# zj15001/PNP_ADMM_CNC_MRI

Measured on AMD Instinct MI355X. Metric: ADMM iterations/sec on 256x256 complex64 slices (batch=512), higher is better.
Workload: dtype f32

## Files before the change

### pnp_admm_cnc_mri_amd/csrc/kernels_slice256.hip

```cpp
#include "engine_host.h"
#include "fused_layout.h"
#include "slice_layout.h"
#include <math.h>
#include <stdio.h>
#include <stdlib.h>
#include <vector>

#ifndef SLICE_EARLY
#define SLICE_EARLY 1
#endif
#ifndef SLICE_PRIOSWAP
#define SLICE_PRIOSWAP 1
#endif
#ifndef SLICE_PRIOMASK
#define SLICE_PRIOMASK 6
#endif
#ifndef SLICE_YH_AUX
#define SLICE_YH_AUX 0
#endif
#ifndef SLICE_ST_AUX
#define SLICE_ST_AUX 0
#endif
#ifndef SLICE_PF
#define SLICE_PF 3
#endif

namespace pnp {

__device__ c32 g_tws[256];

struct SliceArgs {
    float* z;
    float* w;
    float* x;
    const c32* Yh;
    const uint32_t* Mh;
    const c32* Ys;
    const uint32_t* Ms;
    int first, B, iters;
    int slice_xor;
    int flip;
    int state_stride;
    int yh_stride;
    float scale, c;
    ProxParams prox;
    long long* prof;
};

constexpr int RP = 18;
constexpr int REGION = 16 * RP;
constexpr int WREG = 4 * REGION;
constexpr int SL_YS = SL_BUF + REGION;
constexpr int SL_LDS = SL_YS + 256 + 32;
static_assert(SL_WAVES * WREG <= SL_BUF, "wave regions must fit in the buffer they alias");
constexpr int SL4_XB = SL_WAVES * WREG;
constexpr int SL4_YS = SL4_XB + REGION;
constexpr int SL4_RES = SL4_YS + 256 + 32;
__device__ __forceinline__ int sl_lds_float(int set, int q) { return set == 0 ? sl_res_index(0, 0, q) : sl_res1_index(popc8(sl_units_lds(set) & ((1u << q) - 1)), 0, 0); }
constexpr int SL4_LDS = SL4_RES + SL_RES * 256 + SL_NLDS1 * 1024;
static_assert(SL_BUF4 <= SL4_XB && SL4_RES % 2 == 0 && SL4_LDS * 8 <= 160 * 1024, "four-pass LDS map");
template <int PROX> constexpr bool slice_four() { return PROX == 2; }
template <int PROX> constexpr bool slice_res() { return slice_four<PROX>() && SLICE_RESIDENT; }
__device__ __forceinline__ void lds_ld4(const float* p, float (&v)[4]) {
    const float4 q = *reinterpret_cast<const float4*>(p);
    v[0] = q.x; v[1] = q.y; v[2] = q.z; v[3] = q.w;
}
__device__ __forceinline__ void lds_st4(float* p, const float (&v)[4]) { *reinterpret_cast<float4*>(p) = make_float4(v[0], v[1], v[2], v[3]); }

__device__ __forceinline__ void wave_sync() {
    __builtin_amdgcn_fence(__ATOMIC_RELEASE, "wavefront");
    __builtin_amdgcn_wave_barrier();
    __builtin_amdgcn_fence(__ATOMIC_ACQUIRE, "wavefront");
#ifdef SLICE_SYNC_SCHED_BARRIER
    __builtin_amdgcn_sched_barrier(0);
#endif
}

__device__ __forceinline__ void prio_set(int wv, int set) {
#if SLICE_PRIOSWAP
    const bool older_high = (SLICE_PRIOMASK >> set) & 1;
    if (set == 0 || (((SLICE_PRIOMASK >> set) ^ (SLICE_PRIOMASK >> (set - 1))) & 1)) {
        asm volatile("" : "+s"(wv));
        if ((wv < 4) == older_high) __builtin_amdgcn_s_setprio(1); else __builtin_amdgcn_s_setprio(0);
    }
#endif
}

__device__ __forceinline__ int opaque(int v) {
    asm volatile("" : "+v"(v));
    return v;
}
typedef unsigned int u32x4 __attribute__((ext_vector_type(4)));
typedef unsigned int u32x2 __attribute__((ext_vector_type(2)));
typedef __amdgpu_buffer_rsrc_t bufrsrc;
__device__ __forceinline__ bufrsrc make_rsrc(const void* base, unsigned bytes) {
    return __builtin_amdgcn_make_buffer_rsrc(const_cast<void*>(base), 0, (int)bytes, 0x00020000);
}
__device__ __forceinline__ void ld4(bufrsrc r, int voff, int soff, float (&v)[4]) {
    const u32x4 q = __builtin_amdgcn_raw_buffer_load_b128(r, voff, soff, 16);
    v[0] = __uint_as_float(q.x); v[1] = __uint_as_float(q.y); v[2] = __uint_as_float(q.z); v[3] = __uint_as_float(q.w);
}
__device__ __forceinline__ void st4(bufrsrc r, int voff, int soff, const float (&v)[4]) {
    u32x4 q;
    q.x = __float_as_uint(v[0]); q.y = __float_as_uint(v[1]); q.z = __float_as_uint(v[2]); q.w = __float_as_uint(v[3]);
    __builtin_amdgcn_raw_buffer_store_b128(q, r, voff + soff, 0, SLICE_ST_AUX);
}
__device__ __forceinline__ c32 ldc(bufrsrc r, int voff, int soff) {
    const u32x2 q = __builtin_amdgcn_raw_buffer_load_b64(r, voff, soff, 0);
    return mk<float>(__uint_as_float(q.x), __uint_as_float(q.y));
}
struct SliceBufs {
    bufrsrc z, w, x;
    bufrsrc yh, mh, ys, ms;
};

__device__ __forceinline__ void pin(c32& v) { asm volatile("" : "+v"(v.x), "+v"(v.y)); }
__device__ __forceinline__ void mem_fence_compiler() { asm volatile("" ::: "memory"); }

__device__ __forceinline__ float dpp_lane_xor1(float v) {
    return __int_as_float(__builtin_amdgcn_mov_dpp(__float_as_int(v), 0xB1 , 0xF, 0xF, true));
}
__device__ __forceinline__ c32 dpp_lane_xor1(c32 v) { return mk<float>(dpp_lane_xor1(v.x), dpp_lane_xor1(v.y)); }

__device__ __forceinline__ float sub_partner(float a, float b) {
    float r;
    asm("v_subrev_f32_dpp %0, %1, %2 quad_perm:[1,0,3,2] row_mask:0xf bank_mask:0xf bound_ctrl:1" : "=v"(r) : "v"(b), "v"(a));
    return r;
}
__device__ __forceinline__ float add_partner(float a, float b) {
    float r;
    asm("v_add_f32_dpp %0, %1, %2 quad_perm:[1,0,3,2] row_mask:0xf bank_mask:0xf bound_ctrl:1" : "=v"(r) : "v"(b), "v"(a));
    return r;
}

__device__ __forceinline__ float abs_plus(float a, float w) {
    float r;
    asm("v_add_f32_e64 %0, |%1|, %2" : "=v"(r) : "v"(a), "v"(w));
    return r;
}

__device__ __forceinline__ f2 sub2(f2 a, f2 b) {
    f2 r;
    asm("v_pk_add_f32 %0, %1, %2 neg_lo:[0,1] neg_hi:[0,1]" : "=v"(r) : "v"(a), "v"(b));
    return r;
}


template <bool INV>
__device__ __forceinline__ void group_fft256(c32 (&ac)[16], const c32* twl, c32* region, int t) {
    typedef float f4 __attribute__((ext_vector_type(4)));
    const f4* tw4 = reinterpret_cast<const f4*>(twl + RP * t);
    f2* reg2 = reinterpret_cast<f2*>(region);
    f2 a[16];
#pragma unroll
    for (int k = 0; k < 16; ++k) a[k] = to2(ac[k]);
    dft16_pk<INV>(a);
    mem_fence_compiler();
#pragma unroll
    for (int m = 0; m < 4; ++m) {
        const f4 q = tw4[m];
        if (m) a[2 * m] = tmul_v<INV>(a[2 * m], k2(q.x, q.y));
        a[2 * m + 1] = tmul_v<INV>(a[2 * m + 1], k2(q.z, q.w));
    }
    mem_fence_compiler();
#pragma unroll
    for (int m = 4; m < 8; ++m) {
        const f4 q = tw4[m];
        a[2 * m] = tmul_v<INV>(a[2 * m], k2(q.x, q.y));
        a[2 * m + 1] = tmul_v<INV>(a[2 * m + 1], k2(q.z, q.w));
    }
#pragma unroll
    for (int k = 0; k < 16; ++k) reg2[k * RP + t] = a[k];
    wave_sync();
    const f4* row4 = reinterpret_cast<const f4*>(reg2 + t * RP);
#pragma unroll
    for (int m = 0; m < 8; ++m) {
        const f4 q = row4[m];
        a[2 * m] = k2(q.x, q.y);
        a[2 * m + 1] = k2(q.z, q.w);
    }
    wave_sync();
    dft16_pk<INV>(a);
#pragma unroll
    for (int k = 0; k < 16; ++k) ac[k] = from2(a[k]);
}

struct RowLoads {
    float z[8][4], w[8][4];
};
__device__ __forceinline__ int row_set_offset(int set, int wv) { return (32 * set + 4 * wv) * 2048; }
constexpr int ROW_QSTRIDE = 256;

template <int PROX, bool HAS_INV, int Q0, int Q1, bool RESW = false>
__device__ __forceinline__ void issue_row_loads(const SliceBufs& b, RowLoads& L, int soff, int voff, int qbase = 0, int set = 0, const float* resl = nullptr) {
#pragma unroll
    for (int q = qbase + Q0; q < qbase + Q1; ++q) {
        const int vo = voff + ROW_QSTRIDE * q, so = soff;
        const int home = RESW ? w_home(set, q) : W_HBM;
        if (home != W_HBM) {
            ld4(b.z, vo, so, L.z[q]);
            if (home == W_LDS) lds_ld4(resl + sl_lds_float(set, q), L.w[q]);
        } else if (PROX == 3) {
            ld4(b.w, vo, so, L.w[q]);
        } else if (PROX != 0 || !HAS_INV) {
            ld4(b.z, vo, so, L.z[q]);
            ld4(b.w, vo, so, L.w[q]);
        }
    }
}

__device__ __forceinline__ f2 clamp2(f2 a, float c) {
    return k2(__builtin_amdgcn_fmed3f(a.x, -c, c), __builtin_amdgcn_fmed3f(a.y, -c, c));
}
__device__ __forceinline__ f2 fma2(f2 a, f2 b, f2 c) { return __builtin_elementwise_fma(a, b, c); }
__device__ __forceinline__ f2 splat(float v) { return k2(v, v); }
template <int PROX>
__device__ __forceinline__ void prox_pair(f2 u, f2& z, f2& w, const ProxParams& pc) {
    if (PROX == 2) {
        const f2 cz = clamp2(z, pc.ib);
        const f2 t = fma2(splat(pc.c1), z, fma2(splat(pc.c2), u, splat(pc.c3) * cz));
        z = t - clamp2(t, pc.thr);
    } else {
        z = u - clamp2(u, pc.thr);
    }
    w = u - z;
}

template <bool HAS_INV, int PROX, bool HAS_FWD>
__device__ __forceinline__ void pointwise_q(const SliceBufs& b, const ProxParams& pc, int u_first, bool last,
                                            c32& a0, c32& a1, const float (&z_)[4], const float (&w_)[4], int vs,
                                            int home = W_HBM, float* resw = nullptr, float* wq = nullptr) {
    f2 z[2] = {k2(z_[0], z_[1]), k2(z_[2], z_[3])}, w[2] = {k2(w_[0], w_[1]), k2(w_[2], w_[3])};
#define SL_X_PLUS(a_, w_) (HAS_INV ? k2(abs_plus((a_).x, (w_).x), abs_plus((a_).y, (w_).y)) : (w_))
#define SL_ST4(buf, v) { const float q_[4] = {v[0].x, v[0].y, v[1].x, v[1].y}; st4(buf, vs, 0, q_); }
    if (PROX == 3) {
        f2 u[2];
#pragma unroll
        for (int jj = 0; jj < 2; ++jj) {
            if (!u_first) {
                asm volatile("");
                w[jj] = w[jj] - (w[jj] - clamp2(w[jj], pc.thr));
            }
            u[jj] = SL_X_PLUS(jj ? a1 : a0, w[jj]);
            z[jj] = u[jj] - clamp2(u[jj], pc.thr);
            w[jj] = u[jj] - z[jj];
        }
        if (!last) {
            SL_ST4(b.w, u);
        } else {
            SL_ST4(b.z, z);
            SL_ST4(b.w, w);
        }
    }
    if (PROX == 1 || PROX == 2) {
#pragma unroll
        for (int jj = 0; jj < 2; ++jj) prox_pair<PROX>(SL_X_PLUS(jj ? a1 : a0, w[jj]), z[jj], w[jj], pc);
        SL_ST4(b.z, z);
        if (home == W_LDS) { const float q_[4] = {w[0].x, w[0].y, w[1].x, w[1].y}; lds_st4(resw, q_); }
        else if (home == W_REG) { wq[0] = w[0].x; wq[1] = w[0].y; wq[2] = w[1].x; wq[3] = w[1].y; }
        else SL_ST4(b.w, w);
    }
#undef SL_ST4
#undef SL_X_PLUS
    if (HAS_FWD) {
        const f2 v0 = sub2(z[0], w[0]), v1 = sub2(z[1], w[1]);
        a0 = from2(v0);
        a1 = from2(v1);
    }
}

__device__ __forceinline__ void store_x_natural(const SliceBufs& b, const c32 (&a)[16], c32* wreg, int set, int wv, int lane) {
    const int g = lane >> 4, t = lane & 15;
    c32* region = wreg + g * REGION;
#pragma unroll
    for (int j = 0; j < 16; ++j) region[t + 16 * j] = mk<float>(fabsf(a[j].x), fabsf(a[j].y));
    wave_sync();
#pragma unroll
    for (int i = 0; i < 4; ++i) {
        const c32* cell = wreg + i * REGION + 4 * lane;
        const float4 c01 = *reinterpret_cast<const float4*>(cell);
        const float4 c23 = *reinterpret_cast<const float4*>(cell + 2);
        const int vs = 16 * lane + (2 * (32 * set + 4 * wv + i)) * 1024;
        const float xa[4] = {c01.x, c01.z, c23.x, c23.z}, xb[4] = {c01.y, c01.w, c23.y, c23.w};
        st4(b.x, vs, 0, xa);
        st4(b.x, vs + 1024, 0, xb);
    }
    wave_sync();
}

#ifndef SLICE_L1_PF
#define SLICE_L1_PF 8
#endif
template <int PROX> constexpr int row_pf() { return (PROX == 3) ? SLICE_L1_PF : SLICE_PF; }
__device__ __forceinline__ float* res_lane(float* res, int set, int wv, int lane) {
    return set == 0 ? res + sl_res_index(4 * wv + (lane >> 4), lane & 15, 0) : res + SL_RES * 512 + sl_res1_index(0, 4 * wv + (lane >> 4), lane & 15);
}
typedef float ResRegs[SL_NREG > 0 ? SL_NREG : 1][4];
template <int PROX, bool HAS_INV, bool RES = false>
__device__ __forceinline__ void row_phase_prefetch(const SliceBufs& b, RowLoads& L, int wv, int lane, float* res = nullptr) {
    issue_row_loads<PROX, HAS_INV, 0, row_pf<PROX>(), RES>(b, L, row_set_offset(0, wv), 2048 * (lane >> 4) + 16 * (lane & 15), 0, 0, RES ? res_lane(res, 0, wv, lane) : nullptr);
}
template <bool HAS_INV, int PROX, bool HAS_FWD, bool PRELOADED = false, bool RES = false>
__device__ __forceinline__ void row_phase(const SliceBufs& b, const ProxParams& pc, int u_first, bool last, c32 (&F)[SL_SETS][16],
                                          c32* wreg, const c32* twl, int wv, int lane, ResRegs& wr, RowLoads* pre = nullptr, float* res = nullptr) {
    const int g = lane >> 4, t = lane & 15;
    c32* region = wreg + g * REGION;
    const int voff = 2048 * g + 16 * t;
    float* const resl[2] = {RES ? res_lane(res, 0, wv, lane) : nullptr, RES && SL_NLDS1 ? res_lane(res, 1, wv, lane) : nullptr};
    constexpr bool RES_LOOP = RES && HAS_INV;
    constexpr int PF = row_pf<PROX>();
    RowLoads L;
    if (PRELOADED) L = *pre;
    else issue_row_loads<PROX, HAS_INV, 0, PF, RES_LOOP>(b, L, row_set_offset(0, wv), voff, 0, 0, resl[0]);
#pragma unroll
    for (int set = 0; set < SL_SETS; ++set) {
        c32 (&a)[16] = F[set];
        prio_set(wv, set);
        const int soff = row_set_offset(set, wv);
        if (HAS_INV) {
            group_fft256<true>(a, twl, region, t);
        }
        if (HAS_INV && last) store_x_natural(b, a, wreg, set, wv, lane);
        const int vs = voff + soff;
#pragma unroll
        for (int q = 0; q < 8; ++q) {
            const int home = RES ? w_home(set, q) : W_HBM;
            float* const rl = home == W_LDS ? resl[set] + sl_lds_float(set, q) : nullptr;
            float* const wq = wr[home == W_REG ? sl_reg_slot(set, q) : 0];
            if (q + PF < 8) issue_row_loads<PROX, HAS_INV, 0, 1, RES_LOOP>(b, L, soff, voff, q + PF, set, resl[set < 2 ? set : 0]);
            if (RES_LOOP && home != W_HBM) {
                pointwise_q<HAS_INV, PROX, HAS_FWD>(b, pc, u_first, last, a[2 * q], a[2 * q + 1], L.z[q], home == W_REG ? wr[sl_reg_slot(set, q)] : L.w[q],
                                                    vs + ROW_QSTRIDE * q, home, rl, wq);
            } else {
                if (home == W_LDS) lds_st4(rl, L.w[q]);
                if (home == W_REG) { wq[0] = L.w[q][0]; wq[1] = L.w[q][1]; wq[2] = L.w[q][2]; wq[3] = L.w[q][3]; }
                pointwise_q<HAS_INV, PROX, HAS_FWD>(b, pc, u_first, last, a[2 * q], a[2 * q + 1], L.z[q], L.w[q], vs + ROW_QSTRIDE * q);
            }
        }
        if (set + 1 < SL_SETS) issue_row_loads<PROX, HAS_INV, 0, PF, RES_LOOP>(b, L, row_set_offset(set + 1, wv), voff, 0, set + 1, resl[set + 1 < 2 ? set + 1 : 0]);
        if (HAS_FWD) {
            group_fft256<false>(a, twl, region, t);
        }
    }
}

__device__ __forceinline__ void resident_flush(const SliceBufs& b, float* res, const ResRegs& wr, int wv, int lane) {
#pragma unroll
    for (int set = 0; set < SL_SETS; ++set) {
        const int vs = 2048 * (lane >> 4) + 16 * (lane & 15) + row_set_offset(set, wv);
#pragma unroll
        for (int q = 0; q < 8; ++q) {
            const int home = w_home(set, q);
            if (home == W_LDS) {
                float v[4];
                lds_ld4(res_lane(res, set, wv, lane) + sl_lds_float(set, q), v);
                st4(b.w, vs + ROW_QSTRIDE * q, 0, v);
            } else if (home == W_REG) {
                st4(b.w, vs + ROW_QSTRIDE * q, 0, wr[sl_reg_slot(set, q)]);
            }
        }
    }
}

#define SL_PASS0_REGS(X, t)                                                                       \
    X(0, 0, (t)) X(1, 1, (t) + 16) X(2, 2, (t) + 32) X(3, 3, (t) + 48)                              \
    X(12, 8, ((t) ? SL_M + 64 - (t) : SL_M))                                                      \
    X(13, 13, SL_M + 48 - (t)) X(14, 14, SL_M + 32 - (t)) X(15, 15, SL_M + 16 - (t))
#define SL_PASS1_REGS(X, t)                                                                       \
    X(4, 4, (t)) X(5, 5, (t) + 16) X(6, 6, (t) + 32) X(7, 7, (t) + 48)                              \
    X(8, 12, ((t) ? SL_M + 64 - (t) : SL_M))                                                      \
    X(9, 9, SL_M + 48 - (t)) X(10, 10, SL_M + 32 - (t)) X(11, 11, SL_M + 16 - (t))

#define SL_PASS4_REGS(X, t, Q)                                                                    \
    X(2 * (Q), 2 * (Q), (t)) X(2 * (Q) + 1, 2 * (Q) + 1, (t) + 16)                                  \
    X(14 - 2 * (Q), ((Q) ? 16 - 2 * (Q) : 8), ((t) ? SL_M4 + 32 - (t) : SL_M4))                   \
    X(15 - 2 * (Q), 15 - 2 * (Q), SL_M4 + 16 - (t))

__device__ __forceinline__ void lds_put(c32* p, c32 v, bool swapped) {
    float* f = reinterpret_cast<float*>(p);
    if (swapped) { f[0] = v.y; f[1] = v.x; } else { *p = v; }
}
__device__ __forceinline__ c32 lds_get(const c32* p, bool swapped) {
    const float* f = reinterpret_cast<const float*>(p);
    return swapped ? mk<float>(f[1], f[0]) : *p;
}
template <int P, bool FOUR = false>
__device__ __forceinline__ void t_store_rows(const c32 (&F)[16], c32* rp, int t) {
#define SL_T1_STORE(ja, jb, slot) { lds_put(rp + (slot), t ? F[ja] : F[jb], (ja) >= 8); }
    if (FOUR) { SL_PASS4_REGS(SL_T1_STORE, t, P) } else if (P == 0) { SL_PASS0_REGS(SL_T1_STORE, t) } else { SL_PASS1_REGS(SL_T1_STORE, t) }
#undef SL_T1_STORE
}
template <int P, bool FOUR = false>
__device__ __forceinline__ void t_load_rows(c32 (&F)[16], const c32* rp, int t) {
#define SL_T2_LOAD(ja, jb, slot) { F[ja] = lds_get(rp + (slot), (ja) >= 8); }
    if (FOUR) { SL_PASS4_REGS(SL_T2_LOAD, t, P) } else if (P == 0) { SL_PASS0_REGS(SL_T2_LOAD, t) } else { SL_PASS1_REGS(SL_T2_LOAD, t) }
#undef SL_T2_LOAD
    if (FOUR && P == 3) {
        const c32 a8 = F[8];
        F[8] = t ? a8 : F[14];
        F[14] = t ? F[14] : F[12];
        F[12] = t ? F[12] : F[10];
        F[10] = t ? F[10] : a8;
    }
    if (!FOUR && P == 1) {
        const c32 a0 = F[8];
        F[8] = t ? a0 : F[12];
        F[12] = t ? F[12] : a0;
    }
}

template <bool MAYBE_PACKED, int PITCH = SL_P>
__device__ __forceinline__ void t1_read_col(c32 (&Gs)[16], const c32* buf, int off, int odd, bool packed) {
    int off_hi = off + 64 * PITCH;
    asm volatile("" : "+v"(off_hi));
    const c32 *col = buf + off, *col_hi = buf + off_hi;
#pragma unroll
    for (int jb = 0; jb < 16; jb += 8) {
        c32 own[8];
#pragma unroll
        for (int k = 0; k < 8; ++k) own[k] = jb ? col_hi[8 * k * PITCH] : col[8 * k * PITCH];
#pragma unroll
        for (int k = 0; k < 8; ++k) {
            c32 v = mk<float>(add_partner(own[k].x, own[k].y), sub_partner(own[k].y, own[k].x));
            if (MAYBE_PACKED) {
                const float oy = dpp_lane_xor1(own[k].y);
                const c32 raw = mk<float>(odd ? oy : own[k].x, odd ? own[k].x : oy);
                v = packed ? raw : v;
            }
            Gs[jb + k] = v;
            pin(Gs[jb + k]);
        }
    }
}
template <int P>
__device__ __forceinline__ void t1_pass(const c32 (&F)[SL_SETS][16], c32 (&G)[SL_SETS][16], c32* buf, int wv, int lane) {
    const int g = lane >> 4, t = lane & 15;
#pragma unroll
    for (int set = 0; set < SL_SETS; ++set) t_store_rows<P>(F[set], buf + (32 * set + 4 * wv + g) * SL_P, t);
    __syncthreads();
#pragma unroll
    for (int h = 0; h < 2; ++h) {
        const int cc = 32 * h + 4 * wv + g, odd = t & 1;
        const int off = (t >> 1) * SL_P + cc + (odd ? SL_M : 0);
        if (P == 0 && h == 0 && wv == 0) t1_read_col<true>(G[2 * P + h], buf, off, odd, cc == 0);
        else t1_read_col<false>(G[2 * P + h], buf, off, odd, false);
    }
    __syncthreads();
}

template <bool MAYBE_PACKED, int PITCH = SL_P>
__device__ __forceinline__ void t2_write_col(const c32 (&Gs)[16], c32* buf, int off, int odd, bool packed) {
    int off_hi = off + 64 * PITCH;
    asm volatile("" : "+v"(off_hi));
    c32 *col = buf + off, *col_hi = buf + off_hi;
#pragma unroll
    for (int j = 0; j < 16; ++j) {
        const c32 own = Gs[j];
        c32 v = mk<float>(sub_partner(own.x, own.y), add_partner(own.y, own.x));
        if (MAYBE_PACKED) {
            const c32 other = dpp_lane_xor1(own);
            const c32 raw = mk<float>(odd ? own.y : own.x, odd ? other.y : other.x);
            v = packed ? raw : v;
        }
        if (j < 8) col[8 * j * PITCH] = v; else col_hi[8 * (j - 8) * PITCH] = v;
    }
}
template <int P>
__device__ __forceinline__ void t2_pass(const c32 (&G)[SL_SETS][16], c32 (&F)[SL_SETS][16], c32* buf, int wv, int lane) {
    const int g = lane >> 4, t = lane & 15;
#pragma unroll
    for (int h = 0; h < 2; ++h) {
        const int cc = 32 * h + 4 * wv + g, odd = t & 1;
        const int off = (t >> 1) * SL_P + cc + (odd ? SL_M : 0);
        if (P == 0 && h == 0 && wv == 0) t2_write_col<true>(G[2 * P + h], buf, off, odd, cc == 0);
        else t2_write_col<false>(G[2 * P + h], buf, off, odd, false);
    }
    __syncthreads();
#pragma unroll
    for (int set = 0; set < SL_SETS; ++set) t_load_rows<P>(F[set], buf + (32 * set + 4 * wv + g) * SL_P, t);
    __syncthreads();
}

template <int Q>
__device__ __forceinline__ void t1_pass4(const c32 (&F)[SL_SETS][16], c32 (&G)[SL_SETS][16], c32* buf, int wv, int lane) {
    const int g = lane >> 4, t = lane & 15;
#pragma unroll
    for (int set = 0; set < SL_SETS; ++set) t_store_rows<Q, true>(F[set], buf + (32 * set + 4 * wv + g) * SL_P4, t);
    __syncthreads();
    const int cc = 4 * wv + g, odd = t & 1;
    const int off = (t >> 1) * SL_P4 + cc + (odd ? SL_M4 : 0);
    if (Q == 0 && wv == 0) t1_read_col<true, SL_P4>(G[Q], buf, off, odd, cc == 0);
    else t1_read_col<false, SL_P4>(G[Q], buf, off, odd, false);
    __syncthreads();
}
template <int Q>
__device__ __forceinline__ void t2_pass4(const c32 (&G)[SL_SETS][16], c32 (&F)[SL_SETS][16], c32* buf, int wv, int lane) {
    const int g = lane >> 4, t = lane & 15;
    const int cc = 4 * wv + g, odd = t & 1;
    const int off = (t >> 1) * SL_P4 + cc + (odd ? SL_M4 : 0);
    if (Q == 0 && wv == 0) t2_write_col<true, SL_P4>(G[Q], buf, off, odd, cc == 0);
    else t2_write_col<false, SL_P4>(G[Q], buf, off, odd, false);
    __syncthreads();
#pragma unroll
    for (int set = 0; set < SL_SETS; ++set) t_load_rows<Q, true>(F[set], buf + (32 * set + 4 * wv + g) * SL_P4, t);
    __syncthreads();
}

struct ColLoads {
    c32 yh[16];
    uint32_t code;
};
__device__ __forceinline__ void issue_col_loads(const SliceBufs& b, ColLoads& Y, int set, int wv, int lane) {
    const int ybase = (set * 8 + wv) * 8192;
    Y.code = __builtin_amdgcn_raw_buffer_load_b32(b.mh, 4 * lane, (set * 8 + wv) * 64 * 4, 0);
#pragma unroll
    for (int jp = 0; jp < 8; ++jp) {
        const u32x4 q = __builtin_amdgcn_raw_buffer_load_b128(b.yh, 16 * lane + 1024 * (jp & 3), ybase + 4096 * (jp >> 2), SLICE_YH_AUX);
        Y.yh[2 * jp] = mk<float>(__uint_as_float(q.x), __uint_as_float(q.y));
        Y.yh[2 * jp + 1] = mk<float>(__uint_as_float(q.z), __uint_as_float(q.w));
    }
}

__device__ __forceinline__ float code_byte(unsigned m, int byte) {
    float r;
    if (byte == 0) asm("v_cvt_f32_ubyte0 %0, %1" : "=v"(r) : "v"(m));
    else if (byte == 1) asm("v_cvt_f32_ubyte1 %0, %1" : "=v"(r) : "v"(m));
    else if (byte == 2) asm("v_cvt_f32_ubyte2 %0, %1" : "=v"(r) : "v"(m));
    else asm("v_cvt_f32_ubyte3 %0, %1" : "=v"(r) : "v"(m));
    return r;
}
__device__ __forceinline__ void blend_set(c32 (&a)[16], const c32 (&yh)[16], unsigned code, float cs, float chs, float os) {
    const unsigned m[4] = {code & 0x03030303u, (code >> 2) & 0x03030303u, (code >> 4) & 0x03030303u, (code >> 6) & 0x03030303u};
#pragma unroll
    for (int j = 0; j < 16; j += 2) {
        const f2 cf = k2(code_byte(m[j & 3], j >> 2), code_byte(m[(j & 3) + 1], j >> 2));
        const f2 A2 = fma2(splat(-chs), cf, splat(os));
        a[j] = from2(fma2(A2.xx, to2(a[j]), splat(cs) * to2(yh[j])));
        a[j + 1] = from2(fma2(A2.yy, to2(a[j + 1]), splat(cs) * to2(yh[j + 1])));
    }
}

__device__ __forceinline__ void col_phase(const SliceBufs& b, float cdc, float scale, c32 (&G)[SL_SETS][16], c32* wreg, c32* ysl, const c32* twl, int wv, int lane) {
    const int g = lane >> 4, t = lane & 15;
    c32* region = wreg + g * REGION;
    const float cs = cdc * scale, chs = 0.5f * cdc * scale;
    ColLoads Y;
    issue_col_loads(b, Y, 0, wv, lane);
    if (wv == 0) {
        __builtin_amdgcn_raw_ptr_buffer_load_lds(b.ys, ysl, 16, 16 * lane, 0, 0, 0);
        __builtin_amdgcn_raw_ptr_buffer_load_lds(b.ys, ysl + 128, 16, 16 * lane, 1024, 0, 0);
        __builtin_amdgcn_raw_ptr_buffer_load_lds(b.ms, ysl + 256, 4, 4 * lane, 0, 0, 0);
    }
#pragma unroll
    for (int set = 0; set < SL_SETS; ++set) {
        c32 (&a)[16] = G[set];
        prio_set(wv, set);
        group_fft256<false>(a, twl, region, t);
        if (set == 0 && wv == 0 && g == 0) {
#pragma unroll
            for (int j = 0; j < 16; ++j) region[t + 16 * j] = a[j];
            region[256 + t] = a[0];
            wave_sync();
            const uint32_t code_b = reinterpret_cast<const uint32_t*>(ysl + 256)[t];
            const c32* mirror = region + (16 - t);
            const unsigned ma[4] = {Y.code & 0x03030303u, (Y.code >> 2) & 0x03030303u, (Y.code >> 4) & 0x03030303u, (Y.code >> 6) & 0x03030303u};
            const unsigned mb[4] = {code_b & 0x03030303u, (code_b >> 2) & 0x03030303u, (code_b >> 4) & 0x03030303u, (code_b >> 6) & 0x03030303u};
#pragma unroll
            for (int j = 0; j < 16; ++j) {
                const c32 gm = mirror[16 * (15 - j)];
                const c32 A = blend_scaled_f(unpack_a(a[j], gm), Y.yh[j], code_byte(ma[j & 3], j >> 2), cs, chs, scale);
                const c32 Bv = blend_scaled_f(unpack_b(a[j], gm), ysl[t + 16 * j], code_byte(mb[j & 3], j >> 2), cs, chs, scale);
                a[j] = repack_p(A, Bv);
            }
            wave_sync();
        } else {
            blend_set(a, Y.yh, Y.code, cs, 0.5f * chs, 0.5f * scale);
        }
        if (set + 1 < SL_SETS) issue_col_loads(b, Y, set + 1, wv, lane);
        group_fft256<true>(a, twl, region, t);
    }
}

template <int PROX>
__global__ __launch_bounds__(512) void k_slice(SliceArgs p) {
    constexpr bool FOUR = slice_four<PROX>(), RES = slice_res<PROX>();
    __shared__ __attribute__((aligned(16))) c32 lds[FOUR ? SL4_LDS : SL_LDS];
    const int tid = threadIdx.x, lane = tid & 63;
    const int wv = __builtin_amdgcn_readfirstlane(tid >> 6);
    c32* twl = lds + (FOUR ? SL4_XB : SL_BUF);
    c32* ysl = lds + (FOUR ? SL4_YS : SL_YS);
    float* res = RES ? reinterpret_cast<float*>(lds + SL4_RES) : nullptr;
    if (tid < 256) twl[RP * (tid >> 4) + (tid & 15)] = g_tws[((tid >> 4) * (tid & 15)) & 255];
    c32* wreg = lds + wv * WREG;
    __syncthreads();
    for (int sb = blockIdx.x; sb < p.B; sb += gridDim.x) {
        const int sx = ((sb ^ p.slice_xor) < p.B) ? (sb ^ p.slice_xor) : sb;
        const int slice = p.first + (p.flip ? p.B - 1 - sx : sx);
        const size_t so = (size_t)slice * p.state_stride;
        SliceBufs b;
        b.z = make_rsrc(p.z + so, 65536 * 4); b.w = make_rsrc(p.w + so, 65536 * 4); b.x = make_rsrc(p.x + (size_t)slice * 65536, 65536 * 4);
        b.yh = make_rsrc(p.Yh + (size_t)slice * p.yh_stride, YH3_SLICE * 8); b.mh = make_rsrc(p.Mh + (size_t)slice * MH3_SLICE, MH3_SLICE * 4);
        b.ys = make_rsrc(p.Ys + (size_t)slice * 256, 256 * 8); b.ms = make_rsrc(p.Ms + (size_t)slice * 16, 16 * 4);
        c32 F[SL_SETS][16];
        ResRegs wres;
#ifdef SLICE_PROF
        long long* prof = (p.prof && tid == 0 && sb == (int)blockIdx.x) ? p.prof + (size_t)slice * (2 + 6 * p.iters) : nullptr;
#define SL_STAMP() if (prof) *prof++ = wall_clock64()
#else
#define SL_STAMP()
#endif
        SL_STAMP();
        row_phase<false, 0, true, false, RES>(b, p.prox, 1, false, F, wreg, twl, wv, opaque(lane), wres, nullptr, res);
        SL_STAMP();
        for (int it = 0; it < p.iters; ++it) {
            c32 G[SL_SETS][16];
            __syncthreads();
            SL_STAMP();
            if (FOUR) {
                t1_pass4<0>(F, G, lds, wv, opaque(lane));
                t1_pass4<1>(F, G, lds, wv, opaque(lane));
                t1_pass4<2>(F, G, lds, wv, opaque(lane));
                t1_pass4<3>(F, G, lds, wv, opaque(lane));
            } else {
                t1_pass<0>(F, G, lds, wv, opaque(lane));
                t1_pass<1>(F, G, lds, wv, opaque(lane));
            }
#ifdef SLICE_PROF_CLOCK
            if (prof) *prof++ = (long long)__builtin_readcyclecounter();
#else
            SL_STAMP();
#endif
            col_phase(b, p.c, p.scale, G, wreg, ysl, twl, wv, opaque(lane));
            SL_STAMP();
            __syncthreads();
            SL_STAMP();
            if (FOUR) {
                t2_pass4<0>(G, F, lds, wv, opaque(lane));
                t2_pass4<1>(G, F, lds, wv, opaque(lane));
                t2_pass4<2>(G, F, lds, wv, opaque(lane));
            } else {
                t2_pass<0>(G, F, lds, wv, opaque(lane));
            }
#if SLICE_EARLY
            RowLoads L0;
            row_phase_prefetch<PROX, true, RES>(b, L0, wv, opaque(lane), res);
#endif
            if (FOUR) t2_pass4<3>(G, F, lds, wv, opaque(lane));
            else t2_pass<1>(G, F, lds, wv, opaque(lane));
            SL_STAMP();
            const int u_first = (it == 0);
#if SLICE_EARLY
            row_phase<true, PROX, true, true, RES>(b, p.prox, u_first, it + 1 == p.iters, F, wreg, twl, wv, opaque(lane), wres, &L0, res);
#else
            row_phase<true, PROX, true, false, RES>(b, p.prox, u_first, it + 1 == p.iters, F, wreg, twl, wv, opaque(lane), wres, nullptr, res);
#endif
            SL_STAMP();
        }
        if (RES) resident_flush(b, res, wres, wv, opaque(lane));
        __syncthreads();
    }
}

constexpr int SP_P = 17;
__global__ __launch_bounds__(256) void k_sprepare(const c32* y, const uint8_t* mask_bank, const int32_t* mask_id,
                                                  c32* Yh, uint32_t* Mh, c32* Ys, uint32_t* Ms, int yh_stride) {
    __shared__ c32 yd[256 * SP_P], ym[256 * SP_P];
    __shared__ uint8_t md[256 * SP_P], mm[256 * SP_P];
    const int tid = threadIdx.x, m = blockIdx.x, slice = blockIdx.y;
    const int mid = mask_id ? mask_id[slice] : 0;
    const c32* ys = y + (size_t)slice * 65536;
    const uint8_t* ms = mask_bank + (size_t)mid * 65536;
    const int ncol = (m == 8) ? 1 : 16;
#pragma unroll 4
    for (int i = 0; i < 16; ++i) {
        const int idx = tid + 256 * i, r = idx >> 4, c = idx & 15;
        if (c < ncol) {
            const int k2 = 16 * m + c, k2m = (256 - k2) & 255;
            yd[r * SP_P + c] = ys[r * 256 + k2];
            md[r * SP_P + c] = ms[r * 256 + k2];
            ym[r * SP_P + c] = ys[r * 256 + k2m];
            mm[r * SP_P + c] = ms[r * 256 + k2m];
        }
    }
    __syncthreads();
    auto entry = [&](int k1, int c, c32& yh) -> int {
        const int r2 = (256 - k1) & 255;
        const int m1 = md[k1 * SP_P + c] != 0, m2 = mm[r2 * SP_P + c] != 0;
        const c32 y1 = yd[k1 * SP_P + c], y2 = ym[r2 * SP_P + c];
        yh = mk<float>(0.5f * ((m1 ? y1.x : 0.f) + (m2 ? y2.x : 0.f)), 0.5f * ((m1 ? y1.y : 0.f) - (m2 ? y2.y : 0.f)));
        return m1 + m2;
    };
    if (m == 8) {
        c32 yh;
        const int code = entry(tid, 0, yh);
        Ys[(size_t)slice * 256 + tid] = yh;
        __shared__ int codes[256];
        codes[tid] = code;
        __syncthreads();
        if (tid < 16) {
            uint32_t v = 0;
#pragma unroll
            for (int jj = 0; jj < 16; ++jj) v |= (uint32_t)codes[tid + 16 * jj] << (2 * jj);
            Ms[slice * 16 + tid] = v;
        }
        return;
    }
    const int set = m >> 1;
#pragma unroll 4
    for (int i = 0; i < 16; ++i) {
        const int o = tid + 256 * i, blk = o >> 10, e = o & 1023;
        const int jp = e >> 7, lane = (e >> 1) & 63, j = 2 * jp + (e & 1);
        const int g = lane >> 4, t = lane & 15, wv = 4 * (m & 1) + blk;
        c32 yh;
        (void)entry(t + 16 * j, 4 * blk + g, yh);
        Yh[(size_t)slice * yh_stride + yh3_index(0, set, j, wv, lane)] = yh;
    }
    {
        const int blk = tid >> 6, lane = tid & 63, g = lane >> 4, t = lane & 15, wv = 4 * (m & 1) + blk;
        uint32_t v = 0;
#pragma unroll
        for (int j = 0; j < 16; ++j) {
            c32 yh;
            v |= (uint32_t)entry(t + 16 * j, 4 * blk + g, yh) << (2 * j);
        }
        Mh[mh3_index(slice, set, wv, lane)] = v;
    }
}

template <bool TO_SLICE>
__global__ __launch_bounds__(128) void k_state_order(const float* sz, const float* sw, float* dz, float* dw, int src_stride, int dst_stride) {
    __shared__ float tile[2][2048];
    const size_t sbase = (size_t)blockIdx.y * src_stride + (size_t)blockIdx.x * 2048, dbase = (size_t)blockIdx.y * dst_stride + (size_t)blockIdx.x * 2048;
    const float4* pz = reinterpret_cast<const float4*>(sz + sbase);
    const float4* pw = reinterpret_cast<const float4*>(sw + sbase);
    float4* qz = reinterpret_cast<float4*>(dz + dbase);
    float4* qw = reinterpret_cast<float4*>(dw + dbase);
    float4 vz[4], vw[4];
#pragma unroll
    for (int u = 0; u < 4; ++u) { vz[u] = pz[threadIdx.x + 128 * u]; vw[u] = pw[threadIdx.x + 128 * u]; }
#pragma unroll
    for (int u = 0; u < 4; ++u) {
        const int i = threadIdx.x + 128 * u, row = i >> 6, n0 = 4 * (i & 63);
        const float az[4] = {vz[u].x, vz[u].y, vz[u].z, vz[u].w}, aw[4] = {vw[u].x, vw[u].y, vw[u].z, vw[u].w};
#pragma unroll
        for (int k = 0; k < 4; ++k) {
            const int at = TO_SLICE ? (int)sl_state_index(row, n0 + k) : 4 * i + k;
            tile[0][at] = az[k];
            tile[1][at] = aw[k];
        }
    }
    __syncthreads();
#pragma unroll
    for (int u = 0; u < 4; ++u) {
        const int i = threadIdx.x + 128 * u, row = i >> 6, n0 = 4 * (i & 63);
        float oz[4], ow[4];
#pragma unroll
        for (int k = 0; k < 4; ++k) {
            const int at = TO_SLICE ? 4 * i + k : (int)sl_state_index(row, n0 + k);
            oz[k] = tile[0][at];
            ow[k] = tile[1][at];
        }
        qz[i] = make_float4(oz[0], oz[1], oz[2], oz[3]);
        qw[i] = make_float4(ow[0], ow[1], ow[2], ow[3]);
    }
}

struct Slice256 {
    int Bmax = 0, cus = 0;
    int flip = 0;
    int pad = 0, yh_pad = 0;
    float* zs = nullptr;
    float* ws = nullptr;
    float* zprev = nullptr;
    c32* Yh = nullptr;
    uint32_t* Mh = nullptr;
    c32* Ys = nullptr;
    uint32_t* Ms = nullptr;
    SideQueues queues;
};

int slice256_cus(const Slice256* f) { return f && f->cus > 0 ? f->cus : 256; }

hipError_t slice256_state_order(Slice256* f, hipStream_t s, float* z, float* w, int B, bool to_slice) {
    if (B <= 0) return hipSuccess;
    if (f && f->pad > 0) {
        if (to_slice) hipLaunchKernelGGL(k_state_order<true>, dim3(32, B), dim3(128), 0, s, z, w, f->zs, f->ws, 65536, 65536 + f->pad);
        else          hipLaunchKernelGGL(k_state_order<false>, dim3(32, B), dim3(128), 0, s, f->zs, f->ws, z, w, 65536 + f->pad, 65536);
    } else {
        if (to_slice) hipLaunchKernelGGL(k_state_order<true>, dim3(32, B), dim3(128), 0, s, z, w, z, w, 65536, 65536);
        else          hipLaunchKernelGGL(k_state_order<false>, dim3(32, B), dim3(128), 0, s, z, w, z, w, 65536, 65536);
    }
    return hipGetLastError();
}

hipError_t slice256_trace_snapshot(Slice256* f, hipStream_t s, const float* z, int B) {
    const size_t stride = 65536 + (size_t)f->pad;
    if (B > f->Bmax) return hipErrorInvalidValue;
    if (!f->zprev) { hipError_t e = hipMalloc((void**)&f->zprev, (size_t)f->Bmax * stride * sizeof(float)); if (e != hipSuccess) return e; }
    return hipMemcpyAsync(f->zprev, f->pad > 0 ? f->zs : z, (size_t)B * stride * sizeof(float), hipMemcpyDeviceToDevice, s);
}
hipError_t slice256_residuals(Slice256* f, hipStream_t s, const float* x, const float* z, const float* w, const uint8_t* gt, int B,
                              double* partial, unsigned* counter, double* out) {
    if (!f->zprev || B > f->Bmax) return hipErrorInvalidValue;
    return launch_residuals<float>(s, x, f->pad > 0 ? f->zs : z, f->zprev, f->pad > 0 ? f->ws : w, gt, 0, B, 65536, 65536 + (size_t)f->pad, true,
                                   partial, counter, out);
}

// ... 115 lines not shown
```

### pnp_admm_cnc_mri_amd/csrc/slice_layout.h

```cpp
#pragma once
#include <stddef.h>
#include <stdint.h>
#include "fft16.h"

namespace pnp {

constexpr int SL_P = 132;
constexpr int SL_M = 66;
constexpr int SL_BUF = 128 * SL_P;

PNP_HD int sl_pass(int k) { return (k < 64 || k > 192 || k == 128) ? 0 : 1; }
PNP_HD int sl_slot(int k) {
    if (k < 64) return k;
    if (k == 128) return SL_M;
    if (k > 192) return SL_M + 256 - k;
    if (k < 128) return k - 64;
    return SL_M + 192 - k;
}
constexpr int SL_P4 = 68;
constexpr int SL_M4 = 34;
constexpr int SL_BUF4 = 128 * SL_P4;
PNP_HD int sl_pass4(int k) { return k == 128 ? 0 : k < 128 ? (k >> 5) : ((256 - k) >> 5); }
PNP_HD int sl_slot4(int k) { return k == 128 ? SL_M4 : k < 128 ? (k & 31) : SL_M4 + ((256 - k) & 31); }
constexpr int SL_WAVES = 8, SL_SETS = 4;
constexpr int SL_RES = 32;
PNP_HD int sl_res_index(int r, int t, int q) { return 512 * r + 64 * q + 4 * t; }
constexpr int SL_RES1 = 2;
PNP_HD int sl_res1_index(int u, int rr, int t) { return 2048 * u + 64 * rr + 4 * t; }
#ifndef SLICE_RESIDENT
#define SLICE_RESIDENT 1
#endif
#ifndef SLICE_UNITS_LDS1
#define SLICE_UNITS_LDS1 0x03
#endif
#ifndef SLICE_UNITS_REG
#define SLICE_UNITS_REG 0x03000000
#endif
constexpr int popc8(unsigned m) { int n = 0; for (int i = 0; i < 8; ++i) n += (m >> i) & 1; return n; }
constexpr unsigned sl_units_lds(int set) { return SLICE_RESIDENT == 0 ? 0u : set == 0 ? 0xFFu : (SLICE_RESIDENT == 1 && set == 1) ? (SLICE_UNITS_LDS1 & 0xFFu) : 0u; }
constexpr unsigned sl_units_reg(int set) { return SLICE_RESIDENT == 1 && set < SL_SETS ? ((unsigned)SLICE_UNITS_REG >> (8 * set)) & 0xFFu & ~sl_units_lds(set) : 0u; }
enum { W_HBM = 0, W_LDS = 1, W_REG = 2 };
constexpr int w_home(int set, int q) { return ((sl_units_lds(set) >> q) & 1) ? W_LDS : ((sl_units_reg(set) >> q) & 1) ? W_REG : W_HBM; }
constexpr int sl_reg_slot(int set, int q) {
    int n = 0;
    for (int s = 0; s < set; ++s) n += popc8(sl_units_reg(s));
    return n + (set < SL_SETS ? popc8(sl_units_reg(set) & ((1u << q) - 1)) : 0);
}
constexpr int SL_NREG = sl_reg_slot(SL_SETS, 0);
constexpr int SL_NLDS1 = popc8(sl_units_lds(1));
static_assert(SL_NLDS1 <= SL_RES1, "the second resident region holds SL_RES1 units");

PNP_HD int sl_unit(int set, int wv, int lane) { return 32 * set + 4 * wv + (lane >> 4); }

constexpr size_t YH3_SLICE = 4 * 16 * 8 * 64;
constexpr size_t MH3_SLICE = 4 * 8 * 64;
PNP_HD size_t yh3_index(int slice, int set, int j, int wv, int lane) {
    return (size_t)slice * YH3_SLICE + ((((size_t)set * 8 + wv) * 8 + (j >> 1)) * 64 + lane) * 2 + (j & 1);
}
PNP_HD size_t mh3_index(int slice, int set, int wv, int lane) { return (size_t)slice * MH3_SLICE + (((size_t)set * 8 + wv) * 64 + lane); }

PNP_HD size_t sl_state_index(int row, int n) {
    return (size_t)(row >> 1) * 512 + 64 * (n >> 5) + 4 * (n & 15) + 2 * ((n >> 4) & 1) + (row & 1);
}


}
```

Measured before the change: 11210.

## Shrink LDS exchange buffers to free space for more resident state units

The four-pass kernel now does its per-wave FFT transposes and the x store through float-split (real then imaginary) exchange regions, and runs the inter-phase transposes in two half-passes over a 64-row buffer. This roughly halves the LDS footprint of the scratch buffers. The freed LDS holds more of the per-slice w state as resident units (7 instead of 2 in the second region), so less state travels to and from HBM each iteration. The cost is extra wave syncs and block barriers per transpose, plus scalar rather than vector LDS accesses.

```diff
diff --git a/pnp_admm_cnc_mri_amd/csrc/kernels_slice256.hip b/pnp_admm_cnc_mri_amd/csrc/kernels_slice256.hip
--- a/pnp_admm_cnc_mri_amd/csrc/kernels_slice256.hip
+++ b/pnp_admm_cnc_mri_amd/csrc/kernels_slice256.hip
@@ -53,12 +53,8 @@
 constexpr int SL_YS = SL_BUF + REGION;
 constexpr int SL_LDS = SL_YS + 256 + 32;
 static_assert(SL_WAVES * WREG <= SL_BUF, "wave regions must fit in the buffer they alias");
-constexpr int SL4_XB = SL_WAVES * WREG;
-constexpr int SL4_YS = SL4_XB + REGION;
-constexpr int SL4_RES = SL4_YS + 256 + 32;
 __device__ __forceinline__ int sl_lds_float(int set, int q) { return set == 0 ? sl_res_index(0, 0, q) : sl_res1_index(popc8(sl_units_lds(set) & ((1u << q) - 1)), 0, 0); }
-constexpr int SL4_LDS = SL4_RES + SL_RES * 256 + SL_NLDS1 * 1024;
-static_assert(SL_BUF4 <= SL4_XB && SL4_RES % 2 == 0 && SL4_LDS * 8 <= 160 * 1024, "four-pass LDS map");
+static_assert(REGION * 8 == SL2_TW_BYTES && (256 + 32) * 8 == SL2_YS_BYTES && SL2_END % 8 == 0, "tables of the LDS map");
 template <int PROX> constexpr bool slice_four() { return PROX == 2; }
 template <int PROX> constexpr bool slice_res() { return slice_four<PROX>() && SLICE_RESIDENT; }
 __device__ __forceinline__ void lds_ld4(const float* p, float (&v)[4]) {
@@ -146,7 +142,8 @@
 }
 
 
-template <bool INV>
+typedef __attribute__((address_space(3))) float lds_float;
+template <bool INV, bool SPLIT = false>
 __device__ __forceinline__ void group_fft256(c32 (&ac)[16], const c32* twl, c32* region, int t) {
     typedef float f4 __attribute__((ext_vector_type(4)));
     const f4* tw4 = reinterpret_cast<const f4*>(twl + RP * t);
@@ -169,17 +166,31 @@
         a[2 * m] = tmul_v<INV>(a[2 * m], k2(q.x, q.y));
         a[2 * m + 1] = tmul_v<INV>(a[2 * m + 1], k2(q.z, q.w));
     }
-#pragma unroll
-    for (int k = 0; k < 16; ++k) reg2[k * RP + t] = a[k];
-    wave_sync();
-    const f4* row4 = reinterpret_cast<const f4*>(reg2 + t * RP);
-#pragma unroll
-    for (int m = 0; m < 8; ++m) {
-        const f4 q = row4[m];
-        a[2 * m] = k2(q.x, q.y);
-        a[2 * m + 1] = k2(q.z, q.w);
-    }
-    wave_sync();
+    if (SPLIT) {
+        float* rf = reinterpret_cast<float*>(region);
+        const volatile lds_float* row = (const volatile lds_float*)(rf + sl_xw(t, 0));
+#pragma unroll
+        for (int h = 0; h < 2; ++h) {
+#pragma unroll
+            for (int k = 0; k < 16; ++k) rf[sl_xw(k, t)] = h ? a[k].y : a[k].x;
+            wave_sync();
+#pragma unroll
+            for (int k = 0; k < 16; ++k) { if (h) a[k].y = row[k]; else a[k].x = row[k]; }
+            wave_sync();
+        }
+    } else {
+#pragma unroll
+        for (int k = 0; k < 16; ++k) reg2[k * RP + t] = a[k];
+        wave_sync();
+        const f4* row4 = reinterpret_cast<const f4*>(reg2 + t * RP);
+#pragma unroll
+        for (int m = 0; m < 8; ++m) {
+            const f4 q = row4[m];
+            a[2 * m] = k2(q.x, q.y);
+            a[2 * m + 1] = k2(q.z, q.w);
+        }
+        wave_sync();
+    }
     dft16_pk<INV>(a);
 #pragma unroll
     for (int k = 0; k < 16; ++k) ac[k] = from2(a[k]);
@@ -269,8 +280,27 @@
     }
 }
 
+template <bool SPLIT = false>
 __device__ __forceinline__ void store_x_natural(const SliceBufs& b, const c32 (&a)[16], c32* wreg, int set, int wv, int lane) {
     const int g = lane >> 4, t = lane & 15;
+    if (SPLIT) {
+        float* wf = reinterpret_cast<float*>(wreg);
+        float* rf = wf + g * SL_XREGION;
+#pragma unroll
+        for (int h = 0; h < 2; ++h) {
+#pragma unroll
+            for (int j = 0; j < 16; ++j) rf[t + 16 * j] = fabsf(h ? a[j].y : a[j].x);
+            wave_sync();
+#pragma unroll
+            for (int i = 0; i < 4; ++i) {
+                float v[4];
+                lds_ld4(wf + i * SL_XREGION + 4 * lane, v);
+                st4(b.x, 16 * lane + (2 * (32 * set + 4 * wv + i) + h) * 1024, 0, v);
+            }
+            wave_sync();
+        }
+        return;
+    }
     c32* region = wreg + g * REGION;
 #pragma unroll
     for (int j = 0; j < 16; ++j) region[t + 16 * j] = mk<float>(fabsf(a[j].x), fabsf(a[j].y));
@@ -300,11 +330,11 @@
 __device__ __forceinline__ void row_phase_prefetch(const SliceBufs& b, RowLoads& L, int wv, int lane, float* res = nullptr) {
     issue_row_loads<PROX, HAS_INV, 0, row_pf<PROX>(), RES>(b, L, row_set_offset(0, wv), 2048 * (lane >> 4) + 16 * (lane & 15), 0, 0, RES ? res_lane(res, 0, wv, lane) : nullptr);
 }
-template <bool HAS_INV, int PROX, bool HAS_FWD, bool PRELOADED = false, bool RES = false>
+template <bool HAS_INV, int PROX, bool HAS_FWD, bool PRELOADED = false, bool RES = false, bool SPLIT = false>
 __device__ __forceinline__ void row_phase(const SliceBufs& b, const ProxParams& pc, int u_first, bool last, c32 (&F)[SL_SETS][16],
                                           c32* wreg, const c32* twl, int wv, int lane, ResRegs& wr, RowLoads* pre = nullptr, float* res = nullptr) {
     const int g = lane >> 4, t = lane & 15;
-    c32* region = wreg + g * REGION;
+    c32* region = SPLIT ? reinterpret_cast<c32*>(reinterpret_cast<float*>(wreg) + g * SL_XREGION) : wreg + g * REGION;
     const int voff = 2048 * g + 16 * t;
     float* const resl[2] = {RES ? res_lane(res, 0, wv, lane) : nullptr, RES && SL_NLDS1 ? res_lane(res, 1, wv, lane) : nullptr};
     constexpr bool RES_LOOP = RES && HAS_INV;
@@ -318,9 +348,9 @@
         prio_set(wv, set);
         const int soff = row_set_offset(set, wv);
         if (HAS_INV) {
-            group_fft256<true>(a, twl, region, t);
-        }
-        if (HAS_INV && last) store_x_natural(b, a, wreg, set, wv, lane);
+            group_fft256<true, SPLIT>(a, twl, region, t);
+        }
+        if (HAS_INV && last) store_x_natural<SPLIT>(b, a, wreg, set, wv, lane);
         const int vs = voff + soff;
 #pragma unroll
         for (int q = 0; q < 8; ++q) {
@@ -339,7 +369,7 @@
         }
         if (set + 1 < SL_SETS) issue_row_loads<PROX, HAS_INV, 0, PF, RES_LOOP>(b, L, row_set_offset(set + 1, wv), voff, 0, set + 1, resl[set + 1 < 2 ? set + 1 : 0]);
         if (HAS_FWD) {
-            group_fft256<false>(a, twl, region, t);
+            group_fft256<false, SPLIT>(a, twl, region, t);
         }
     }
 }
@@ -409,28 +439,30 @@
     }
 }
 
+template <bool MAYBE_PACKED, int PITCH>
+__device__ __forceinline__ void t1_read_col8(c32 (&Gs)[16], int jb, const c32* col, int odd, bool packed) {
+    c32 own[8];
+#pragma unroll
+    for (int k = 0; k < 8; ++k) own[k] = col[8 * k * PITCH];
+#pragma unroll
+    for (int k = 0; k < 8; ++k) {
+        c32 v = mk<float>(add_partner(own[k].x, own[k].y), sub_partner(own[k].y, own[k].x));
+        if (MAYBE_PACKED) {
+            const float oy = dpp_lane_xor1(own[k].y);
+            const c32 raw = mk<float>(odd ? oy : own[k].x, odd ? own[k].x : oy);
+            v = packed ? raw : v;
+        }
+        Gs[jb + k] = v;
+        pin(Gs[jb + k]);
+    }
+}
 template <bool MAYBE_PACKED, int PITCH = SL_P>
 __device__ __forceinline__ void t1_read_col(c32 (&Gs)[16], const c32* buf, int off, int odd, bool packed) {
     int off_hi = off + 64 * PITCH;
     asm volatile("" : "+v"(off_hi));
     const c32 *col = buf + off, *col_hi = buf + off_hi;
-#pragma unroll
-    for (int jb = 0; jb < 16; jb += 8) {
-        c32 own[8];
-#pragma unroll
-        for (int k = 0; k < 8; ++k) own[k] = jb ? col_hi[8 * k * PITCH] : col[8 * k * PITCH];
-#pragma unroll
-        for (int k = 0; k < 8; ++k) {
-            c32 v = mk<float>(add_partner(own[k].x, own[k].y), sub_partner(own[k].y, own[k].x));
-            if (MAYBE_PACKED) {
-                const float oy = dpp_lane_xor1(own[k].y);
-                const c32 raw = mk<float>(odd ? oy : own[k].x, odd ? own[k].x : oy);
-                v = packed ? raw : v;
-            }
-            Gs[jb + k] = v;
-            pin(Gs[jb + k]);
-        }
-    }
+    t1_read_col8<MAYBE_PACKED, PITCH>(Gs, 0, col, odd, packed);
+    t1_read_col8<MAYBE_PACKED, PITCH>(Gs, 8, col_hi, odd, packed);
 }
 template <int P>
 __device__ __forceinline__ void t1_pass(const c32 (&F)[SL_SETS][16], c32 (&G)[SL_SETS][16], c32* buf, int wv, int lane) {
@@ -448,13 +480,10 @@
     __syncthreads();
 }
 
-template <bool MAYBE_PACKED, int PITCH = SL_P>
-__device__ __forceinline__ void t2_write_col(const c32 (&Gs)[16], c32* buf, int off, int odd, bool packed) {
-    int off_hi = off + 64 * PITCH;
-    asm volatile("" : "+v"(off_hi));
-    c32 *col = buf + off, *col_hi = buf + off_hi;
-#pragma unroll
-    for (int j = 0; j < 16; ++j) {
+template <bool MAYBE_PACKED, int PITCH>
+__device__ __forceinline__ void t2_write_col8(const c32 (&Gs)[16], int jb, c32* col, int odd, bool packed) {
+#pragma unroll
+    for (int j = jb; j < jb + 8; ++j) {
         const c32 own = Gs[j];
         c32 v = mk<float>(sub_partner(own.x, own.y), add_partner(own.y, own.x));
         if (MAYBE_PACKED) {
@@ -462,8 +491,16 @@
             const c32 raw = mk<float>(odd ? own.y : own.x, odd ? other.y : other.x);
             v = packed ? raw : v;
         }
-        if (j < 8) col[8 * j * PITCH] = v; else col_hi[8 * (j - 8) * PITCH] = v;
-    }
+        col[8 * (j - jb) * PITCH] = v;
+    }
+}
+template <bool MAYBE_PACKED, int PITCH = SL_P>
+__device__ __forceinline__ void t2_write_col(const c32 (&Gs)[16], c32* buf, int off, int odd, bool packed) {
+    int off_hi = off + 64 * PITCH;
+    asm volatile("" : "+v"(off_hi));
+    c32 *col = buf + off, *col_hi = buf + off_hi;
+    t2_write_col8<MAYBE_PACKED, PITCH>(Gs, 0, col, odd, packed);
+    t2_write_col8<MAYBE_PACKED, PITCH>(Gs, 8, col_hi, odd, packed);
 }
 template <int P>
 __device__ __forceinline__ void t2_pass(const c32 (&G)[SL_SETS][16], c32 (&F)[SL_SETS][16], c32* buf, int wv, int lane) {
@@ -482,28 +519,34 @@
 }
 
 template <int Q>
-__device__ __forceinline__ void t1_pass4(const c32 (&F)[SL_SETS][16], c32 (&G)[SL_SETS][16], c32* buf, int wv, int lane) {
-    const int g = lane >> 4, t = lane & 15;
-#pragma unroll
-    for (int set = 0; set < SL_SETS; ++set) t_store_rows<Q, true>(F[set], buf + (32 * set + 4 * wv + g) * SL_P4, t);
-    __syncthreads();
-    const int cc = 4 * wv + g, odd = t & 1;
-    const int off = (t >> 1) * SL_P4 + cc + (odd ? SL_M4 : 0);
-    if (Q == 0 && wv == 0) t1_read_col<true, SL_P4>(G[Q], buf, off, odd, cc == 0);
-    else t1_read_col<false, SL_P4>(G[Q], buf, off, odd, false);
-    __syncthreads();
-}
-template <int Q>
-__device__ __forceinline__ void t2_pass4(const c32 (&G)[SL_SETS][16], c32 (&F)[SL_SETS][16], c32* buf, int wv, int lane) {
+__device__ __forceinline__ void t1_pass8(const c32 (&F)[SL_SETS][16], c32 (&G)[SL_SETS][16], c32* buf, int wv, int lane) {
     const int g = lane >> 4, t = lane & 15;
     const int cc = 4 * wv + g, odd = t & 1;
-    const int off = (t >> 1) * SL_P4 + cc + (odd ? SL_M4 : 0);
-    if (Q == 0 && wv == 0) t2_write_col<true, SL_P4>(G[Q], buf, off, odd, cc == 0);
-    else t2_write_col<false, SL_P4>(G[Q], buf, off, odd, false);
-    __syncthreads();
-#pragma unroll
-    for (int set = 0; set < SL_SETS; ++set) t_load_rows<Q, true>(F[set], buf + (32 * set + 4 * wv + g) * SL_P4, t);
-    __syncthreads();
+    const c32* col = buf + (t >> 1) * SL_P4 + cc + (odd ? SL_M4 : 0);
+#pragma unroll
+    for (int h = 0; h < 2; ++h) {
+#pragma unroll
+        for (int s = 0; s < 2; ++s) t_store_rows<Q, true>(F[2 * h + s], buf + sl_row8(32 * (2 * h + s) + 4 * wv + g) * SL_P4, t);
+        __syncthreads();
+        if (Q == 0 && wv == 0) t1_read_col8<true, SL_P4>(G[Q], 8 * h, col, odd, cc == 0);
+        else t1_read_col8<false, SL_P4>(G[Q], 8 * h, col, odd, false);
+        __syncthreads();
+    }
+}
+template <int Q>
+__device__ __forceinline__ void t2_pass8(const c32 (&G)[SL_SETS][16], c32 (&F)[SL_SETS][16], c32* buf, int wv, int lane) {
+    const int g = lane >> 4, t = lane & 15;
+    const int cc = 4 * wv + g, odd = t & 1;
+    c32* col = buf + (t >> 1) * SL_P4 + cc + (odd ? SL_M4 : 0);
+#pragma unroll
+    for (int h = 0; h < 2; ++h) {
+        if (Q == 0 && wv == 0) t2_write_col8<true, SL_P4>(G[Q], 8 * h, col, odd, cc == 0);
+        else t2_write_col8<false, SL_P4>(G[Q], 8 * h, col, odd, false);
+        __syncthreads();
+#pragma unroll
+        for (int s = 0; s < 2; ++s) t_load_rows<Q, true>(F[2 * h + s], buf + sl_row8(32 * (2 * h + s) + 4 * wv + g) * SL_P4, t);
+        __syncthreads();
+    }
 }
 
 struct ColLoads {
@@ -540,9 +583,10 @@
     }
 }
 
+template <bool SPLIT = false>
 __device__ __forceinline__ void col_phase(const SliceBufs& b, float cdc, float scale, c32 (&G)[SL_SETS][16], c32* wreg, c32* ysl, const c32* twl, int wv, int lane) {
     const int g = lane >> 4, t = lane & 15;
-    c32* region = wreg + g * REGION;
+    c32* region = SPLIT ? reinterpret_cast<c32*>(reinterpret_cast<float*>(wreg) + g * SL_XREGION) : wreg + g * REGION;
     const float cs = cdc * scale, chs = 0.5f * cdc * scale;
     ColLoads Y;
     issue_col_loads(b, Y, 0, wv, lane);
@@ -555,7 +599,7 @@
     for (int set = 0; set < SL_SETS; ++set) {
         c32 (&a)[16] = G[set];
         prio_set(wv, set);
-        group_fft256<false>(a, twl, region, t);
+        group_fft256<false, SPLIT>(a, twl, region, t);
         if (set == 0 && wv == 0 && g == 0) {
 #pragma unroll
             for (int j = 0; j < 16; ++j) region[t + 16 * j] = a[j];
@@ -577,21 +621,21 @@
             blend_set(a, Y.yh, Y.code, cs, 0.5f * chs, 0.5f * scale);
         }
         if (set + 1 < SL_SETS) issue_col_loads(b, Y, set + 1, wv, lane);
-        group_fft256<true>(a, twl, region, t);
+        group_fft256<true, SPLIT>(a, twl, region, t);
     }
 }
 
 template <int PROX>
 __global__ __launch_bounds__(512) void k_slice(SliceArgs p) {
     constexpr bool FOUR = slice_four<PROX>(), RES = slice_res<PROX>();
-    __shared__ __attribute__((aligned(16))) c32 lds[FOUR ? SL4_LDS : SL_LDS];
+    __shared__ __attribute__((aligned(16))) c32 lds[FOUR ? SL2_END / 8 : SL_LDS];
     const int tid = threadIdx.x, lane = tid & 63;
     const int wv = __builtin_amdgcn_readfirstlane(tid >> 6);
-    c32* twl = lds + (FOUR ? SL4_XB : SL_BUF);
-    c32* ysl = lds + (FOUR ? SL4_YS : SL_YS);
-    float* res = RES ? reinterpret_cast<float*>(lds + SL4_RES) : nullptr;
+    c32* twl = lds + (FOUR ? SL2_TW / 8 : SL_BUF);
+    c32* ysl = lds + (FOUR ? SL2_YS / 8 : SL_YS);
+    float* res = RES ? reinterpret_cast<float*>(lds + SL2_RES0 / 8) : nullptr;
     if (tid < 256) twl[RP * (tid >> 4) + (tid & 15)] = g_tws[((tid >> 4) * (tid & 15)) & 255];
-    c32* wreg = lds + wv * WREG;
+    c32* wreg = FOUR ? reinterpret_cast<c32*>(reinterpret_cast<float*>(lds) + wv * SL_XWAVE) : lds + wv * WREG;
     __syncthreads();
     for (int sb = blockIdx.x; sb < p.B; sb += gridDim.x) {
         const int sx = ((sb ^ p.slice_xor) < p.B) ? (sb ^ p.slice_xor) : sb;
@@ -610,17 +654,17 @@
 #define SL_STAMP()
 #endif
         SL_STAMP();
-        row_phase<false, 0, true, false, RES>(b, p.prox, 1, false, F, wreg, twl, wv, opaque(lane), wres, nullptr, res);
+        row_phase<false, 0, true, false, RES, FOUR>(b, p.prox, 1, false, F, wreg, twl, wv, opaque(lane), wres, nullptr, res);
         SL_STAMP();
         for (int it = 0; it < p.iters; ++it) {
             c32 G[SL_SETS][16];
             __syncthreads();
             SL_STAMP();
             if (FOUR) {
-                t1_pass4<0>(F, G, lds, wv, opaque(lane));
-                t1_pass4<1>(F, G, lds, wv, opaque(lane));
-                t1_pass4<2>(F, G, lds, wv, opaque(lane));
-                t1_pass4<3>(F, G, lds, wv, opaque(lane));
+                t1_pass8<0>(F, G, lds, wv, opaque(lane));
+                t1_pass8<1>(F, G, lds, wv, opaque(lane));
+                t1_pass8<2>(F, G, lds, wv, opaque(lane));
+                t1_pass8<3>(F, G, lds, wv, opaque(lane));
             } else {
                 t1_pass<0>(F, G, lds, wv, opaque(lane));
                 t1_pass<1>(F, G, lds, wv, opaque(lane));
@@ -630,14 +674,14 @@
 #else
             SL_STAMP();
 #endif
-            col_phase(b, p.c, p.scale, G, wreg, ysl, twl, wv, opaque(lane));
+            col_phase<FOUR>(b, p.c, p.scale, G, wreg, ysl, twl, wv, opaque(lane));
             SL_STAMP();
             __syncthreads();
             SL_STAMP();
             if (FOUR) {
-                t2_pass4<0>(G, F, lds, wv, opaque(lane));
-                t2_pass4<1>(G, F, lds, wv, opaque(lane));
-                t2_pass4<2>(G, F, lds, wv, opaque(lane));
+                t2_pass8<0>(G, F, lds, wv, opaque(lane));
+                t2_pass8<1>(G, F, lds, wv, opaque(lane));
+                t2_pass8<2>(G, F, lds, wv, opaque(lane));
             } else {
                 t2_pass<0>(G, F, lds, wv, opaque(lane));
             }
@@ -645,14 +689,14 @@
             RowLoads L0;
             row_phase_prefetch<PROX, true, RES>(b, L0, wv, opaque(lane), res);
 #endif
-            if (FOUR) t2_pass4<3>(G, F, lds, wv, opaque(lane));
+            if (FOUR) t2_pass8<3>(G, F, lds, wv, opaque(lane));
             else t2_pass<1>(G, F, lds, wv, opaque(lane));
             SL_STAMP();
             const int u_first = (it == 0);
 #if SLICE_EARLY
-            row_phase<true, PROX, true, true, RES>(b, p.prox, u_first, it + 1 == p.iters, F, wreg, twl, wv, opaque(lane), wres, &L0, res);
+            row_phase<true, PROX, true, true, RES, FOUR>(b, p.prox, u_first, it + 1 == p.iters, F, wreg, twl, wv, opaque(lane), wres, &L0, res);
 #else
-            row_phase<true, PROX, true, false, RES>(b, p.prox, u_first, it + 1 == p.iters, F, wreg, twl, wv, opaque(lane), wres, nullptr, res);
+            row_phase<true, PROX, true, false, RES, FOUR>(b, p.prox, u_first, it + 1 == p.iters, F, wreg, twl, wv, opaque(lane), wres, nullptr, res);
 #endif
             SL_STAMP();
         }
diff --git a/pnp_admm_cnc_mri_amd/csrc/slice_layout.h b/pnp_admm_cnc_mri_amd/csrc/slice_layout.h
--- a/pnp_admm_cnc_mri_amd/csrc/slice_layout.h
+++ b/pnp_admm_cnc_mri_amd/csrc/slice_layout.h
@@ -25,13 +25,16 @@
 constexpr int SL_WAVES = 8, SL_SETS = 4;
 constexpr int SL_RES = 32;
 PNP_HD int sl_res_index(int r, int t, int q) { return 512 * r + 64 * q + 4 * t; }
-constexpr int SL_RES1 = 2;
+#ifndef SLICE_RES1_UNITS
+#define SLICE_RES1_UNITS 7
+#endif
+constexpr int SL_RES1 = SLICE_RES1_UNITS;
 PNP_HD int sl_res1_index(int u, int rr, int t) { return 2048 * u + 64 * rr + 4 * t; }
 #ifndef SLICE_RESIDENT
 #define SLICE_RESIDENT 1
 #endif
 #ifndef SLICE_UNITS_LDS1
-#define SLICE_UNITS_LDS1 0x03
+#define SLICE_UNITS_LDS1 0x7F
 #endif
 #ifndef SLICE_UNITS_REG
 #define SLICE_UNITS_REG 0x03000000
@@ -50,6 +53,23 @@
 constexpr int SL_NLDS1 = popc8(sl_units_lds(1));
 static_assert(SL_NLDS1 <= SL_RES1, "the second resident region holds SL_RES1 units");
 
+constexpr int SL_XP = 17;
+constexpr int SL_XREGION = 16 * SL_XP;
+constexpr int SL_XWAVE = 4 * SL_XREGION;
+PNP_HD int sl_xw(int k, int t) { return SL_XP * k + t; }
+constexpr int SL_BUF8 = 64 * SL_P4;
+PNP_HD int sl_row8(int r) { return r & 63; }
+constexpr int sl_max(int a, int b) { return a > b ? a : b; }
+constexpr int SL2_XB = 0,             SL2_XB_BYTES = sl_max(SL_WAVES * SL_XWAVE * 4, SL_BUF8 * 8);
+constexpr int SL2_TW = SL2_XB + SL2_XB_BYTES,     SL2_TW_BYTES = 16 * 18 * 8;
+constexpr int SL2_YS = SL2_TW + SL2_TW_BYTES,     SL2_YS_BYTES = (256 + 32) * 8;
+constexpr int SL2_RES0 = SL2_YS + SL2_YS_BYTES,   SL2_RES0_BYTES = SL_RES * 2048;
+constexpr int SL2_RES1 = SL2_RES0 + SL2_RES0_BYTES, SL2_RES1_BYTES = SL_RES1 * 8192;
+constexpr int SL2_END = SL2_RES1 + SL2_RES1_BYTES;
+constexpr int SL_LDS_CU = 163840;
+static_assert(SL2_END <= SL_LDS_CU && SL2_TW % 16 == 0 && SL2_RES0 % 16 == 0, "LDS map of k_slice<2>");
+static_assert(2 * SL_XREGION >= 272 && SL_XREGION >= 256 && SL_XREGION % 4 == 0, "what else lives in the exchange regions");
+
 PNP_HD int sl_unit(int set, int wv, int lane) { return 32 * set + 4 * wv + (lane >> 4); }
 
 constexpr size_t YH3_SLICE = 4 * 16 * 8 * 64;
```

New measurement: 11820, median of 6. +5.5%, better.
